# IONIQ6000/av1-go

Hardware: AMD Instinct MI355X
Metric: encoded 4K30 frames/sec (whole node) at fixed QP; PSNR-Y delta vs libaom (higher is better)
Workload: dtype u16

## Files before the change

av1-go_amd/csrc/av1_entropy_kernels.hip:

```cpp
#include <string.h>
#include <vector>
#include "av1_ops_cdfs.hpp"
#include "av1_ops8.hpp"
#include "av1mi_internal.hpp"

namespace av1mi {
using namespace av1ops;

struct Av1EntLaunch {
  FrameView fv;
  int nframes, sbr_n, sbc_n;
  BlockInfo *info;
  op_t *ops; uint32_t ops_cap;
  uint32_t *grouped; uint32_t grouped_cap;
  uint16_t *slot_total, *slot_base;
  uint16_t *rec;
  uint32_t *nops;
  uint8_t *slots; uint32_t slot_cap;
  uint32_t *tile_size;
  uint64_t *tile_off;
  uint32_t *status;
  uint8_t *out; uint64_t out_cap;
  const uint16_t *cdf_image; int cdf_words;
  SlotTable tab;
  const uint16_t *cdf_image32; SlotTable tab32;
  const uint8_t *lr_on_frame;
  int sb_rows32, band, nslots;
};

template <int kKey = -1> __device__ __forceinline__ FrameView frame_view(const Av1EntLaunch &L, int f) {
  FrameView v = L.fv;
  const long nb = (long)v.w8 * v.h8;
  if (kKey < 0 ? v.key != 0 : kKey != 0) { v.y_mode += nb * f; v.uv_mode += nb * f; }
  else { v.mv += nb * 2 * f; v.skip += nb * f; }
  v.lev_y += nb * 64 * f; v.lev_u += nb * 16 * f; v.lev_v += nb * 16 * f;
  v.info = L.info + nb * f;
  if (L.lr_on_frame) for (int p = 0; p < 3; p++) v.lr_on[p] = v.lr_on[p] && L.lr_on_frame[f * 3 + p];
  return v;
}

__global__ __launch_bounds__(256) void k_av1_info(Av1EntLaunch L) {
  const long nb = (long)L.fv.w8 * L.fv.h8, i = (long)blockIdx.x * 256 + threadIdx.x;
  if (i >= nb * L.nframes) return;
  const int f = (int)(i / nb), b = (int)(i - (long)f * nb);
  const FrameView v = frame_view<0>(L, f);
  BlockInfo o = {};
  inter_mode_decision(v, b / v.w8, b % v.w8, &o);
  L.info[nb * f + b] = o;
}

struct TileWave {
  template <class T> using Var = LaneVar<T, 1>;
  template <class F> __device__ __forceinline__ void each(F f) { f((int)threadIdx.x); __syncthreads(); }
  __device__ __forceinline__ int scan(Var<int> &v) {
    const int lane = (int)threadIdx.x, x = v.v[0];
    int inc = x;
#pragma unroll
    for (int d = 1; d < 64; d <<= 1) {
      const int y = __shfl_up(inc, d, 64);
      if (lane >= d) inc += y;
    }
    v.v[0] = inc - x;
    return __shfl(inc, 63, 64);
  }
  __device__ __forceinline__ int first(Var<int> &v) { return __shfl(v.v[0], 0, 64); }
};

__global__ __launch_bounds__(64) __attribute__((amdgpu_waves_per_eu(2, 8))) void k_av1_tokens(Av1EntLaunch L) {
  const int tiles = L.sbr_n * L.sbc_n, t = blockIdx.x, f = t / tiles, tt = t - f * tiles, sbr = tt / L.sbc_n, sbc = tt - sbr * L.sbc_n;
  if (sbr < L.sb_rows32) return;
  const FrameView v = frame_view(L, f);
  __shared__ Tile8Mem S;
  const int below = tiles - L.sb_rows32 * L.sbc_n;
  uint16_t *rec = L.rec + ((size_t)f * below + (tt - (tiles - below))) * kBlocksPerTile * kBlockRecords;
  TileWave w;
  const int n = tok_tile8(w, S, v, sbr, sbc, rec, L.ops + (size_t)t * L.ops_cap, L.ops_cap, L.grouped + (size_t)t * L.grouped_cap,
                          L.slot_total + (size_t)t * S_MAX, L.slot_base + (size_t)t * S_MAX);
  if (threadIdx.x == 0) {
    if (n < 0) atomicOr(L.status, 1u);
    L.nops[t] = n < 0 ? 0u : (uint32_t)n;
  }
}

__global__ __launch_bounds__(64) void k_av1_tokens32(Av1EntLaunch L) {
  __shared__ Tile32Mem S;
  const int tiles = L.sbr_n * L.sbc_n, band = L.sb_rows32 * L.sbc_n, f = blockIdx.x / band, tt = blockIdx.x - f * band, sbr = tt / L.sbc_n, sbc = tt - sbr * L.sbc_n;
  const size_t t = (size_t)f * tiles + tt;
  const FrameView v = frame_view<1>(L, f);
  TileWave w;
  const int n = tok_tile32(w, S, v, sbr, sbc, L.ops + t * L.ops_cap, L.ops_cap, L.grouped + t * L.grouped_cap, L.slot_total + t * S_MAX, L.slot_base + t * S_MAX);
  if (threadIdx.x == 0) {
    if (n < 0) atomicOr(L.status, 1u);
    L.nops[t] = n < 0 ? 0u : (uint32_t)n;
  }
}

__global__ __launch_bounds__(64) void k_av1_chains(Av1EntLaunch L, int ntiles_all, int ngroups) {
  const int xcd = blockIdx.x & 7, j = blockIdx.x >> 3, nslots = L.nslots;
  const int g = (j / nslots) * 8 + xcd, sl = j - (j / nslots) * nslots, lane = threadIdx.x, t = g * 64 + lane;
  if (g >= ngroups) return;
  __shared__ __attribute__((aligned(16))) uint16_t s_big[64 * 16];
  const int n = L.tab.nsym[sl], off = L.tab.off[sl];
  int cnt = 0, base = 0;
  bool mine = t < ntiles_all;
  if (mine && L.band) { const int tiles = L.sbr_n * L.sbc_n, sbr = (t % tiles) / L.sbc_n; mine = (sbr < L.sb_rows32) == (L.band == 1); }
  if (mine) { cnt = L.slot_total[(size_t)t * S_MAX + sl]; base = L.slot_base[(size_t)t * S_MAX + sl]; }
  if (!__any(cnt > 0)) return;
  const size_t tt = t < ntiles_all ? (size_t)t : 0;
  op_t *list = L.ops + tt * L.ops_cap;
  const uint32_t *grouped = L.grouped + tt * L.grouped_cap + base;
  if (n <= 4) {
    const uint32_t *iw = reinterpret_cast<const uint32_t *>(L.cdf_image) + (off >> 1);
    uint64_t cdf = (uint64_t)iw[0] | ((uint64_t)iw[1] << 32);
    const uint4 *g4 = reinterpret_cast<const uint4 *>(grouped);
    const uint4 z = make_uint4(0, 0, 0, 0);
    uint4 c0 = cnt > 0 ? g4[0] : z, c1 = cnt > 4 ? g4[1] : z, c2 = cnt > 8 ? g4[2] : z, c3 = cnt > 12 ? g4[3] : z;
    auto four = [&](const uint4 &v, int e) {
      if (e < cnt) list[v.x >> 4] = small_step(cdf, (int)(v.x & 15), n);
      if (e + 1 < cnt) list[v.y >> 4] = small_step(cdf, (int)(v.y & 15), n);
      if (e + 2 < cnt) list[v.z >> 4] = small_step(cdf, (int)(v.z & 15), n);
      if (e + 3 < cnt) list[v.w >> 4] = small_step(cdf, (int)(v.w & 15), n);
    };
#pragma unroll 1
    for (int e = 0; e < cnt; e += 16) {
      const uint4 *nx = g4 + (e >> 2) + 4;
      const uint4 n0 = e + 16 < cnt ? nx[0] : z, n1 = e + 20 < cnt ? nx[1] : z, n2 = e + 24 < cnt ? nx[2] : z, n3 = e + 28 < cnt ? nx[3] : z;
      four(c0, e); four(c1, e + 4); four(c2, e + 8); four(c3, e + 12);
      c0 = n0; c1 = n1; c2 = n2; c3 = n3;
    }
  } else {
    uint16_t *cdf = s_big + lane * 16;
    {
      const uint4 *iw = reinterpret_cast<const uint4 *>(L.cdf_image + off);
      uint4 *d = reinterpret_cast<uint4 *>(cdf);
      d[0] = iw[0];
      d[1] = n > 8 ? iw[1] : make_uint4(0, 0, 0, 0);
    }
#pragma unroll 1
    for (int e = 0; e < cnt; e++) {
      const uint32_t v = grouped[e];
      const int s = (int)(v & 15);
      list[v >> 4] = s >= kSplitHorz ? split_tuple(cdf, s) : big_step(cdf, s, n);
    }
  }
}

constexpr int kRingOps = 64, kLaneWords = kRingOps * 2 + Coder::kStage + 8;

__global__ __launch_bounds__(64) void k_av1_code(Av1EntLaunch L, int ntiles_all) {
  __shared__ __attribute__((aligned(16))) uint16_t s_lane[64 * kLaneWords];
  const int lane = threadIdx.x, t = blockIdx.x * 64 + lane;
  const bool live = t < ntiles_all;
  uint32_t *ring = reinterpret_cast<uint32_t *>(s_lane + lane * kLaneWords);
  Coder c;
  c.init(L.slots + (size_t)(live ? t : 0) * L.slot_cap, (int)L.slot_cap, s_lane + lane * kLaneWords + kRingOps * 2);
  const int n = live ? (int)L.nops[t] : 0;
  const uint4 *ops4 = reinterpret_cast<const uint4 *>(L.ops + (size_t)(live ? t : 0) * L.ops_cap);
  uint4 r0, r1, r2, r3, r4, r5, r6, r7;
  r0 = r1 = r2 = r3 = r4 = r5 = r6 = r7 = make_uint4(0, 0, 0, 0);
  int w = 0;
  bool pend = false;
  auto request = [&]() {
    const uint4 *p = ops4 + (w >> 2);
    if (w < n) r0 = p[0];
    if (w + 4 < n) r1 = p[1];
    if (w + 8 < n) r2 = p[2];
    if (w + 12 < n) r3 = p[3];
    if (w + 16 < n) r4 = p[4];
    if (w + 20 < n) r5 = p[5];
    if (w + 24 < n) r6 = p[6];
    if (w + 28 < n) r7 = p[7];
    pend = w < n;
  };
  auto take = [&]() {
    uint4 *q = reinterpret_cast<uint4 *>(ring + (w & 32));
    q[0] = r0; q[1] = r1; q[2] = r2; q[3] = r3; q[4] = r4; q[5] = r5; q[6] = r6; q[7] = r7;
    w += 32;
  };
  request();
  if (pend) { take(); request(); }
  int i = 0, lit_left = 0;
  uint32_t op = ring[0], op_next = ring[1], op_next2 = ring[2];
  for (;;) {
    if (!__any(lit_left > 0 || i < n)) break;
    if (__any((pend && w - i < 24) || c.ns >= Coder::kStage - 8)) {
      if (pend && w - i <= 32) { take(); request(); }
      c.spill();
    }
#pragma unroll
    for (int q = 0; q < 8; q++) {
      if (lit_left > 0 || i < n) {
        const uint32_t fetched = ring[(i + 3) & (kRingOps - 1)];
        uint32_t tup = op;
        if (lit_left == 0 && (op >> 31)) lit_left = (int)((op >> 27) & 15);
        if (lit_left > 0) {
          lit_left--;
          tup = (op >> lit_left) & 1 ? (1u << 19) | (256u << 9) : (2u << 19) | (512u << 9) | 256u;
        }
        c.encode_tuple(tup);
        if (lit_left == 0) { i++; op = op_next; op_next = op_next2; op_next2 = fetched; }
      }
    }
  }
  if (!live) return;
  int sz = n ? c.finish() : -1;
  if (sz < 0) { if (n) atomicOr(L.status, 2u); sz = 0; }
  L.tile_size[t] = (uint32_t)sz;
}

__global__ __launch_bounds__(1024) void k_av1_scan(Av1EntLaunch L, int ntiles_all) {
// ... 17 lines not shown
  }
}
__global__ __launch_bounds__(64) void k_av1_gather(Av1EntLaunch L) {
  const int t = blockIdx.x;
  const uint32_t n = L.tile_size[t];
  const uint64_t off = L.tile_off[t];
  if (off + n > L.out_cap) return;
  const uint8_t *src = L.slots + (size_t)t * L.slot_cap;
  uint8_t *dst = L.out + off;
  const uint32_t head = min(n, (uint32_t)((16 - (reinterpret_cast<uintptr_t>(dst) & 15)) & 15)), body = (n - head) >> 4, tail0 = head + (body << 4);
  if (threadIdx.x < head) dst[threadIdx.x] = src[threadIdx.x];
  for (uint32_t i = threadIdx.x; i < body; i += 64) {
    uint4 v;
    __builtin_memcpy(&v, src + head + 16 * i, 16);
    *reinterpret_cast<uint4 *>(dst + head + 16 * i) = v;
  }
  if (tail0 + threadIdx.x < n) dst[tail0 + threadIdx.x] = src[tail0 + threadIdx.x];
}

hipError_t launch_av1_front(av1mi_ctx *ctx, const Av1EntLaunch &L, hipStream_t s) {
  const long nb = (long)L.fv.w8 * L.fv.h8 * L.nframes;
  const int ntiles_all = L.sbr_n * L.sbc_n * L.nframes, ngroups = (ntiles_all + 63) / 64;
  ProfToken t = ctx_prof_begin(ctx, AV1MI_K_ENTROPY_TOKENS, s);
  if (!L.fv.key) hipLaunchKernelGGL(k_av1_info, dim3((unsigned)((nb + 255) / 256)), dim3(256), 0, s, L);
  if (L.sb_rows32 < L.sbr_n) hipLaunchKernelGGL(k_av1_tokens, dim3((unsigned)ntiles_all), dim3(64), 0, s, L);
  if (L.sb_rows32) hipLaunchKernelGGL(k_av1_tokens32, dim3((unsigned)(L.sb_rows32 * L.sbc_n * L.nframes)), dim3(64), 0, s, L);
  ctx_prof_end(ctx, t, s);
  t = ctx_prof_begin(ctx, AV1MI_K_ENTROPY_CHAINS, s);
  Av1EntLaunch C = L;
  C.nslots = L.fv.key ? S_KEY_END : S_INTER_END; C.band = L.sb_rows32 ? 2 : 0;
  if (L.sb_rows32 < L.sbr_n) hipLaunchKernelGGL(k_av1_chains, dim3((unsigned)(((ngroups + 7) / 8) * 8 * C.nslots)), dim3(64), 0, s, C, ntiles_all, ngroups);
  if (L.sb_rows32) {
    C.nslots = K_END; C.band = 1; C.tab = L.tab32; C.cdf_image = L.cdf_image32;
    hipLaunchKernelGGL(k_av1_chains, dim3((unsigned)(((ngroups + 7) / 8) * 8 * C.nslots)), dim3(64), 0, s, C, ntiles_all, ngroups);
  }
  ctx_prof_end(ctx, t, s);
  return hipGetLastError();
}
hipError_t launch_av1_back(av1mi_ctx *ctx, const Av1EntLaunch &L, hipStream_t s) {
  const int ntiles_all = L.sbr_n * L.sbc_n * L.nframes;
  ProfToken t = ctx_prof_begin(ctx, AV1MI_K_ENTROPY, s);
  hipLaunchKernelGGL(k_av1_code, dim3((unsigned)((ntiles_all + 63) / 64)), dim3(64), 0, s, L, ntiles_all);
  ctx_prof_end(ctx, t, s);
  t = ctx_prof_begin(ctx, AV1MI_K_ENTROPY_PACK, s);
  hipLaunchKernelGGL(k_av1_scan, dim3(1), dim3(1024), 0, s, L, ntiles_all);
  hipLaunchKernelGGL(k_av1_gather, dim3((unsigned)ntiles_all), dim3(64), 0, s, L);
  ctx_prof_end(ctx, t, s);
  return hipGetLastError();
}

}

struct av1mi_av1ent_state {
  void *info = nullptr, *ops[2] = { nullptr, nullptr }, *nops[2] = { nullptr, nullptr }, *grouped = nullptr, *slot_tb = nullptr, *rec = nullptr, *slots = nullptr, *tile_off = nullptr, *status = nullptr;
  size_t info_b = 0, ops_b[2] = { 0, 0 }, nops_b[2] = { 0, 0 }, grouped_b = 0, slot_tb_b = 0, rec_b = 0, slots_b = 0, off_b = 0;
  hipEvent_t lists_ready[2] = { nullptr, nullptr }, lists_free[2] = { nullptr, nullptr };
  bool free_recorded[2] = { false, false };
  unsigned long jobs = 0;
  av1mi::Av1EntLaunch pending[2];
  uint64_t *pending_total[2] = { nullptr, nullptr };
  bool pending_valid[2] = { false, false };
  size_t last_tiles = 0;
  uint16_t *d_image[2][4] = {};
  uint16_t *d_image32[4] = {};
  av1ops::SlotTable tab32;
  int image_words[2] = { 0, 0 };
  av1ops::SlotTable tab[2];
};

namespace {
int grow(av1mi_ctx *ctx, void **p, size_t *have, size_t need) {
  if (*have >= need) return AV1MI_OK;
  if (*p) (void)hipFree(*p);
  *p = nullptr; *have = 0;
  if (hipMalloc(p, need) != hipSuccess) return av1mi::ctx_fail(ctx, AV1MI_E_NOMEM, "AV1 entropy scratch: hipMalloc(%zu) failed", need);
  *have = need;
  return AV1MI_OK;
}
}

extern "C" {

uint32_t av1mi_av1_entropy_ops_per_tile(void) { return 32768; }
uint32_t av1mi_av1_entropy_slot_bytes(void) { return 16384; }

}

int av1mi::av1_entropy_front(av1mi_ctx *ctx, const av1mi_av1_entropy_job *j, hipStream_t front, int *ticket) {
  if (!ctx || !ticket) return AV1MI_E_INVAL;
  *ticket = -1;
  if (!j) return av1mi::ctx_fail(ctx, AV1MI_E_INVAL, "null job");
  if (hipSetDevice(av1mi::ctx_device(ctx)) != hipSuccess) return av1mi::ctx_fail(ctx, AV1MI_E_DEVICE, "hipSetDevice failed");
  if (j->width <= 0 || j->height <= 0 || (j->width & 7) || (j->height & 7) || j->width > 4096 || j->height > 4096)
    return av1mi::ctx_fail(ctx, AV1MI_E_INVAL, "frame %dx%d must be a multiple of 8, at most 4096x4096", j->width, j->height);
  if (j->nframes < 0 || j->nframes > 4096 || j->base_q_idx < 1 || j->base_q_idx > 255) return av1mi::ctx_fail(ctx, AV1MI_E_INVAL, "bad nframes / base_q_idx");
  const void *need[] = { j->d_lev_y, j->d_lev_u, j->d_lev_v, j->d_out, j->d_tile_size, j->d_total, j->key ? (const void *)j->d_modes_y : (const void *)j->d_mvs,
                         j->key ? (const void *)j->d_modes_uv : (const void *)j->d_skip };
  for (const void *p : need) if (!p) return av1mi::ctx_fail(ctx, AV1MI_E_INVAL, "null device pointer");
  if (j->nframes == 0) return AV1MI_OK;
  av1mi_av1ent_state *st = av1mi::ctx_av1ent(ctx);
  if (!st) return av1mi::ctx_fail(ctx, AV1MI_E_NOMEM, "AV1 entropy state");
  const int key = j->key ? 1 : 0, qcat = av1ops::q_category(j->base_q_idx);
  if (!st->d_image[key][qcat]) {
    av1ops::SlotTable tab;
    const std::vector<uint16_t> img = av1ops::default_slot_image(key != 0, qcat, &tab);
    st->tab[key] = tab; st->image_words[key] = tab.words;
    if (hipMalloc((void **)&st->d_image[key][qcat], img.size() * 2) != hipSuccess ||
        hipMemcpy(st->d_image[key][qcat], img.data(), img.size() * 2, hipMemcpyHostToDevice) != hipSuccess)
      return av1mi::ctx_fail(ctx, AV1MI_E_DEVICE, "uploading the default CDF image failed");
  }
  if (j->key_rows32 && (!key || (j->key_rows32 & 63) || j->key_rows32 > j->height || (j->width & 31)))
    return av1mi::ctx_fail(ctx, AV1MI_E_INVAL, "key_rows32 %d: whole superblock rows of a key frame whose width is a multiple of 32", j->key_rows32);
  if (j->key_rows32 && !st->d_image32[qcat]) {
    const std::vector<uint16_t> img = av1ops::default_slot_image_k32(qcat, &st->tab32);
    if (hipMalloc((void **)&st->d_image32[qcat], img.size() * 2) != hipSuccess ||
        hipMemcpy(st->d_image32[qcat], img.data(), img.size() * 2, hipMemcpyHostToDevice) != hipSuccess)
      return av1mi::ctx_fail(ctx, AV1MI_E_DEVICE, "uploading the default CDF image failed");
  }
  av1mi::Av1EntLaunch L;
  memset(&L, 0, sizeof(L));
  L.sb_rows32 = j->key_rows32 / 64;
  if (j->key_rows32) { L.tab32 = st->tab32; L.cdf_image32 = st->d_image32[qcat]; }
  L.fv.w8 = j->width / 8; L.fv.h8 = j->height / 8; L.fv.key = key;
  L.fv.y_mode = j->d_modes_y; L.fv.uv_mode = j->d_modes_uv; L.fv.mv = j->d_mvs; L.fv.skip = j->d_skip;
  L.fv.lev_y = j->d_lev_y; L.fv.lev_u = j->d_lev_u; L.fv.lev_v = j->d_lev_v;
  for (int p = 0; p < 3; p++) {
    L.fv.lr_on[p] = j->lr_on[p] != 0;
    const int vh = j->visible_height ? j->visible_height : j->height, vw = j->visible_width ? j->visible_width : j->width;
    const int ph = p ? (vh + 1) / 2 : vh, pw = p ? (vw + 1) / 2 : vw;
    L.fv.lr_rows[p] = (ph + 32) / 64 > 1 ? (ph + 32) / 64 : 1; L.fv.lr_cols[p] = (pw + 32) / 64 > 1 ? (pw + 32) / 64 : 1;
  }
  memcpy(L.fv.lr_unit[0], j->lr_unit_y, 8); memcpy(L.fv.lr_unit[1], j->lr_unit_uv, 8);
  L.nframes = j->nframes; L.sbr_n = (L.fv.h8 + 7) / 8; L.sbc_n = (L.fv.w8 + 7) / 8;
  const size_t nb = (size_t)L.fv.w8 * L.fv.h8 * j->nframes, nt = (size_t)L.sbr_n * L.sbc_n * j->nframes;
  L.ops_cap = av1mi_av1_entropy_ops_per_tile(); L.slot_cap = av1mi_av1_entropy_slot_bytes();
  L.grouped_cap = L.ops_cap + av1ops::kListAlign * av1ops::S_MAX;
  const int par = (int)(st->jobs++ & 1);
  st->last_tiles = nt;
  int rc;
  if ((rc = grow(ctx, &st->info, &st->info_b, nb * sizeof(av1ops::BlockInfo))) ||
      (rc = grow(ctx, &st->ops[par], &st->ops_b[par], nt * L.ops_cap * sizeof(av1ops::op_t))) || (rc = grow(ctx, &st->nops[par], &st->nops_b[par], nt * 4)) ||
      (rc = grow(ctx, &st->grouped, &st->grouped_b, nt * L.grouped_cap * sizeof(uint32_t))) ||
      (rc = grow(ctx, &st->slot_tb, &st->slot_tb_b, nt * av1ops::S_MAX * 4)) ||
      (rc = grow(ctx, &st->rec, &st->rec_b, (size_t)(L.sbr_n - L.sb_rows32) * L.sbc_n * j->nframes * av1ops::kBlocksPerTile * av1ops::kBlockRecords * sizeof(uint16_t))) ||
      (rc = grow(ctx, &st->slots, &st->slots_b, nt * L.slot_cap)) || (rc = grow(ctx, &st->tile_off, &st->off_b, (nt + 1) * 8)))
    return rc;
  L.info = (av1ops::BlockInfo *)st->info; L.ops = (av1ops::op_t *)st->ops[par]; L.nops = (uint32_t *)st->nops[par]; L.grouped = (uint32_t *)st->grouped;
  L.slot_total = (uint16_t *)st->slot_tb; L.slot_base = L.slot_total + nt * av1ops::S_MAX; L.rec = (uint16_t *)st->rec; L.slots = (uint8_t *)st->slots;
  L.tile_off = (uint64_t *)st->tile_off;
  L.tile_size = j->d_tile_size; L.out = j->d_out; L.out_cap = j->out_cap;
  L.status = (uint32_t *)(j->d_total + 1);
  L.cdf_image = st->d_image[key][qcat]; L.cdf_words = st->image_words[key]; L.tab = st->tab[key];
  L.lr_on_frame = j->d_lr_on;
#define E_HIP(call) do { const hipError_t e_ = (call); if (e_ != hipSuccess) return av1mi::ctx_fail(ctx, AV1MI_E_DEVICE, "%s: %s", #call, hipGetErrorString(e_)); } while (0)
  for (hipEvent_t *ev : { &st->lists_ready[par], &st->lists_free[par] }) if (!*ev) E_HIP(hipEventCreateWithFlags(ev, hipEventDisableTiming));
  if (st->free_recorded[par]) E_HIP(hipStreamWaitEvent(front, st->lists_free[par], 0));
  E_HIP(hipMemsetAsync(j->d_total, 0, 16, front));
  E_HIP(av1mi::launch_av1_front(ctx, L, front));
  E_HIP(hipEventRecord(st->lists_ready[par], front));
  st->pending[par] = L; st->pending_total[par] = j->d_total; st->pending_valid[par] = true;
  *ticket = par;
  return AV1MI_OK;
}

int av1mi::av1_entropy_back(av1mi_ctx *ctx, int ticket, hipStream_t back) {
  if (!ctx || ticket < 0 || ticket > 1) return AV1MI_E_INVAL;
  av1mi_av1ent_state *st = av1mi::ctx_av1ent(ctx);
  if (!st || !st->pending_valid[ticket]) return av1mi::ctx_fail(ctx, AV1MI_E_INVAL, "no entropy job pending under this ticket");
  const av1mi::Av1EntLaunch &L = st->pending[ticket];
  const size_t nt = (size_t)L.sbr_n * L.sbc_n * L.nframes;
  E_HIP(hipStreamWaitEvent(back, st->lists_ready[ticket], 0));
  E_HIP(av1mi::launch_av1_back(ctx, L, back));
  E_HIP(hipMemcpyAsync(st->pending_total[ticket], L.tile_off + nt, 8, hipMemcpyDeviceToDevice, back));
  E_HIP(hipEventRecord(st->lists_free[ticket], back)); st->free_recorded[ticket] = true;
  st->pending_valid[ticket] = false;
#undef E_HIP
  return AV1MI_OK;
}

int av1mi::av1_entropy_submit(av1mi_ctx *ctx, const av1mi_av1_entropy_job *j, hipStream_t front, hipStream_t back) {
  int ticket = -1;
  const int rc = av1_entropy_front(ctx, j, front, &ticket);
  if (rc != AV1MI_OK || ticket < 0) return rc;
  return av1_entropy_back(ctx, ticket, back);
}

extern "C" {

int av1mi_av1_entropy_encode_on(av1mi_ctx *ctx, const av1mi_av1_entropy_job *j, void *stream_handle) {
  if (!ctx) return AV1MI_E_INVAL;
  hipStream_t s = stream_handle ? (hipStream_t)stream_handle : av1mi::ctx_stream(ctx);
  return av1mi::av1_entropy_submit(ctx, j, s, s);
}

int av1mi_av1_entropy_encode(av1mi_ctx *ctx, const av1mi_av1_entropy_job *j) { return av1mi_av1_entropy_encode_on(ctx, j, nullptr); }

int av1mi_av1_entropy_last_list_words(av1mi_ctx *ctx, uint64_t *words) {
  if (!ctx || !words) return AV1MI_E_INVAL;
  *words = 0;
  av1mi_av1ent_state *st = av1mi::ctx_av1ent(ctx);
  if (!st || !st->jobs || !st->last_tiles) return AV1MI_OK;
  if (hipSetDevice(av1mi::ctx_device(ctx)) != hipSuccess || hipDeviceSynchronize() != hipSuccess) return av1mi::ctx_fail(ctx, AV1MI_E_DEVICE, "synchronising failed");
  std::vector<uint32_t> n(st->last_tiles);
  if (hipMemcpy(n.data(), st->nops[(st->jobs - 1) & 1], n.size() * 4, hipMemcpyDeviceToHost) != hipSuccess) return av1mi::ctx_fail(ctx, AV1MI_E_DEVICE, "reading the list sizes failed");
  for (uint32_t v : n) *words += v;
  return AV1MI_OK;
}

}

namespace av1mi {
void av1ent_free(av1mi_av1ent_state *st) {
  if (!st) return;
  for (void *p : { st->info, st->ops[0], st->ops[1], st->nops[0], st->nops[1], st->grouped, st->slot_tb, st->rec, st->slots, st->tile_off }) if (p) (void)hipFree(p);
  for (hipEvent_t ev : { st->lists_ready[0], st->lists_ready[1], st->lists_free[0], st->lists_free[1] }) if (ev) (void)hipEventDestroy(ev);
  for (auto &k : st->d_image) for (uint16_t *p : k) if (p) (void)hipFree(p);
  for (uint16_t *p : st->d_image32) if (p) (void)hipFree(p);
  delete st;
}
av1mi_av1ent_state *av1ent_new() { return new (std::nothrow) av1mi_av1ent_state(); }
}
```

av1-go_amd/csrc/av1_ops32.hpp:

```cpp
#pragma once
#include "av1_ops.hpp"

namespace av1ops {

enum SlotK32 : int {
  K_SKIP = 0,
  K_PART32 = 1,
  K_PART64 = 2,
  K_USE_WIENER = 3,
  K_TXB_SKIP_Y = 4,
  K_TXB_SKIP_C = 5,
  K_EOB_Y = 8,
  K_EOB_C = 9,
  K_EOBX_Y = 10,
  K_EOBX_C = 19,
  K_DC_SIGN_Y = 26,
  K_DC_SIGN_C = 29,
  K_BASE_EOB_Y = 32,
  K_BASE_EOB_C = 36,
  K_BASE_Y = 40,
  K_BASE_C = 66,
  K_BR_Y = 92,
  K_BR_C = 113,
  K_KF_Y_MODE = 134,
// ... 210 lines not shown
      uint8_t *col = reinterpret_cast<uint8_t *>(S.round) + lane;
      for (int rs = 0; rs < kRoundSlots; rs++) col[rs * (kRoundStride * 4)] = 0;
      if (lane < nr) {
        CountSink32 k = { col, chroma, 0 };
        R::pass1(k, S, lev, b, p, eob, nr - 1 - lane);
        c = k.n;
      }
    }
    opened[lane] = o; n[lane] = c + o;
  });
  const int words1 = w.scan(n);
  typename W::template Var<RoundCounts> cnt;
  const int nd = (nr + 3) >> 2;
  w.each([&](int lane) {
    if (lane >= kRoundSlots) return;
    RoundCounts &c = cnt[lane];
    AV1_UNROLL
    for (int q = 0; q < kLanes32 / 4; q++) c.w[q] = q < nd ? S.round[lane * kRoundStride + q] : 0u;
  });
  w.each([&](int lane) {
    if (lane >= kRoundSlots) return;
    const RoundCounts &c = cnt[lane];
    const int slot = round_slot_global(lane, chroma);
    uint32_t run = S.run[slot];
    AV1_UNROLL
    for (int q = 0; q < kLanes32 / 4; q++) {
      if (q >= nd) continue;
      const uint32_t u = c.w[q], p0 = run, p1 = p0 + (u & 0xFF), p2 = p1 + ((u >> 8) & 0xFF), p3 = p2 + ((u >> 16) & 0xFF);
      run = p3 + (u >> 24);
      S.round[lane * kRoundStride + 2 * q] = p0 | (p1 << 16); S.round[lane * kRoundStride + 2 * q + 1] = p2 | (p3 << 16);
    }
    S.run[slot] = run;
  });
  w.each([&](int lane) {
    if (lane >= nr) return;
    EmitSink32 k = { reinterpret_cast<u16a *>(S.round) + lane, chroma, words + n[lane] + opened[lane], list, grouped };
    R::pass1(k, S, lev, b, p, eob, nr - 1 - lane);
  });
  words += words1;
  w.each([&](int lane) {
    WordSink32 k = { 0 };
    if (lane < nr) R::pass2(k, S, lev, b, p, eob, lane);
    n[lane] = k.n;
  });
  const int words2 = w.scan(n);
  w.each([&](int lane) {
    if (lane >= nr) return;
    DirectSink32 k = { S.run, words + n[lane], list, grouped };
    R::pass2(k, S, lev, b, p, eob, lane);
  });
  return words + words2;
}

template <class W>
AV1_HD int tok_tile32(W &w, Tile32Mem &S, const FrameView &f, int sbr, int sbc, op_t *list, uint32_t ops_cap, uint32_t *grouped, uint16_t *slot_total,
                      uint16_t *slot_base) {
  typedef typename W::template Var<int> LaneInt;
  const bool half = sbc * 8 + 4 >= f.w8;
  w.each([&](int lane) {
    fill_scan_tables32(&S.scan, lane, kLanes32);
    for (int i = lane; i < kTile32MagBytes / 4; i += kLanes32) reinterpret_cast<u32a *>(S.mag)[i] = 0;
    for (int i = lane; i < K_END; i += kLanes32) S.run[i] = 0;
    if (lane < kBlocks32 * 3) { S.eob[lane] = 0; S.cul[lane] = 0; }
  });
  w.each([&](int lane) {
    AV1_UNROLL
    for (int b = 0; b < kBlocks32; b++) {
      if (half && (b & 1)) continue;
      const long i = block_index32(f, sbr, sbc, b);
      int eob = 0, cul = 0;
      MagMap<32> Y(tile_scratch32(S, b, 0));
      eob = Y.load8(f.lev_y + i * 1024, lane, &cul);
      eob = imax(eob, Y.load8(f.lev_y + i * 1024, lane + kLanes32, &cul));
      if (cul) { AV1_SHARED_MAX(&S.eob[b * 3], eob); AV1_SHARED_ADD(&S.cul[b * 3], cul); }
      const int p = 1 + (lane >> 5);
      MagMap<16> C(tile_scratch32(S, b, p));
      cul = 0;
      eob = C.load8((p == 1 ? f.lev_u : f.lev_v) + i * 256, lane & 31, &cul);
      if (cul) { AV1_SHARED_MAX(&S.eob[b * 3 + p], eob); AV1_SHARED_ADD(&S.cul[b * 3 + p], cul); }
    }
  });
  LaneInt n;
  w.each([&](int lane) {
    TotalSink32 k = { S.run, 0 };
    for (int b = 0; b < kBlocks32; b++) {
      if (half && (b & 1)) continue;
      tok_tb32_total<32>(f, k, S, lane, sbr, sbc, b, 0, half);
      tok_tb32_total<16>(f, k, S, lane, sbr, sbc, b, 1, half);
      tok_tb32_total<16>(f, k, S, lane, sbr, sbc, b, 2, half);
    }
    n[lane] = k.n;
  });
  const int words = w.scan(n);
  enum { kOwn = (K_END + kLanes32 - 1) / kLanes32 };
  w.each([&](int lane) {
    int mine = 0;
    for (int q = 0; q < kOwn; q++) if (lane * kOwn + q < K_END) mine += (int)((S.run[lane * kOwn + q] + kListAlign - 1) & ~(uint32_t)(kListAlign - 1));
    n[lane] = mine;
  });
  const int entries = w.scan(n);
  const bool fits = (uint32_t)words <= ops_cap && entries <= 65535;
  w.each([&](int lane) {
    uint32_t run = (uint32_t)n[lane];
    for (int q = 0; q < kOwn; q++) {
      const int sl = lane * kOwn + q;
      if (sl >= K_END) break;
      const uint32_t tot = S.run[sl];
      slot_total[sl] = (uint16_t)(fits ? tot : 0u); slot_base[sl] = (uint16_t)(fits ? run : 0u);
      S.run[sl] = run;
      run += (tot + kListAlign - 1) & ~(uint32_t)(kListAlign - 1);
    }
    for (int sl = K_END + lane; sl < S_MAX; sl += kLanes32) { slot_total[sl] = 0; slot_base[sl] = 0; }
  });
  if (!fits) return -1;
  int at = 0;
  for (int b = 0; b < kBlocks32; b++) {
    if (half && (b & 1)) continue;
    at = tok_tb32_emit<32>(w, S, f, sbr, sbc, b, 0, half, at, list, grouped);
    at = tok_tb32_emit<16>(w, S, f, sbr, sbc, b, 1, half, at, list, grouped);
    at = tok_tb32_emit<16>(w, S, f, sbr, sbc, b, 2, half, at, list, grouped);
  }
  return at;
}

}
```

av1-go_amd/csrc/av1_ops8.hpp:

```cpp
#pragma once
#include "av1_ops32.hpp"

namespace av1ops {

enum { kLanes8 = kBlocksPerTile, kReplaySlots = (S_MAX + 1) / 2, kOwn8 = (S_MAX + kLanes8 - 1) / kLanes8 };
static_assert(2 * kReplaySlots >= S_MAX && S_MAX <= 256 && kOwn8 * kLanes8 >= S_MAX && 4 * kLanes8 >= S_MAX, "rows are bytes; two passes cover every slot");

struct Tile8Mem {
  union {
    struct { uint8_t cnt[S_MAX * kBlocksPerTile]; alignas(16) uint8_t mag[kBlocksPerTile * kMagBytes]; } p1;
    uint16_t pos[kReplaySlots * kBlocksPerTile];
  };
  uint16_t total[S_MAX], base[S_MAX];
  uint8_t row[(S_MAX + 3) & ~3];
  uint8_t sums[kBlocksPerTile];
  ScanTables scan;
};
struct SlotCounts8 { uint32_t w[kOwn8][kBlocksPerTile / 4]; };

AV1_HD void replay_block8(const uint16_t *rec, int nrec, uint16_t *pos, const uint8_t *row, int blk, int first, op_t *list, uint32_t *grouped, int row_lo,
                          bool literals) {
  int n = first;
  for (int i0 = 0; i0 < nrec; i0 += 8) {
    struct alignas(16) R8 { uint32_t w[4]; } q = *reinterpret_cast<const R8 *>(rec + i0);
    AV1_UNROLL
    for (int j = 0; j < 8; j++, n++) {
      if (i0 + j >= nrec) break;
      const unsigned r = (q.w[j >> 1] >> (16 * (j & 1))) & 0xFFFFu;
      if (r & 0x8000u) { if (literals) list[n] = op_lit((int)((r >> 11) & 15), r & 0x7FFu); }
      else {
        const unsigned rw = (unsigned)row[r >> 4] - (unsigned)row_lo;
        if (rw < (unsigned)kReplaySlots) { uint16_t &p = pos[rw * kBlocksPerTile + blk]; grouped[p] = ((uint32_t)n << 4) | (r & 15u); p++; }
      }
    }
  }
}

template <class W>
AV1_HD int tok_tile8(W &w, Tile8Mem &S, const FrameView &f, int sbr, int sbc, uint16_t *rec, op_t *list, uint32_t ops_cap, uint32_t *grouped,
                     uint16_t *slot_total, uint16_t *slot_base) {
  typedef typename W::template Var<int> LaneInt;
  const int nslots = f.key ? S_KEY_END : S_INTER_END;
  w.each([&](int lane) {
    for (int i = lane; i < S_MAX * kBlocksPerTile / 4; i += kLanes8) reinterpret_cast<u32a *>(S.p1.cnt)[i] = 0;
    if (lane == 0) fill_scan_tables(&S.scan);
    int bx, by;
    demorton8((unsigned)lane, &bx, &by);
    const int r8 = sbr * 8 + by, c8 = sbc * 8 + bx;
    S.sums[by * 8 + bx] = (uint8_t)(r8 < f.h8 && c8 < f.w8 ? block_levels_summary(f, r8 * f.w8 + c8) : 0u);
  });
  LaneInt nrec, first;
  w.each([&](int lane) {
    const TokScratch ts = { S.p1.mag + lane * kMagBytes, &S.scan };
    Sink k = { rec + (size_t)lane * kBlockRecords, S.p1.cnt, lane, 0, 0, false };
    tok_block(f, k, ts, sbr, sbc, lane, S.sums);
    nrec[lane] = k.nrec;
    first[lane] = k.n | (k.overflow ? 1 << 24 : 0);
  });
  const int sum = w.scan(first), words = sum & 0xFFFFFF;
  bool fits = (uint32_t)words <= ops_cap && !(sum >> 24);
  typename W::template Var<SlotCounts8> cnt;
  if (fits) w.each([&](int lane) {
    SlotCounts8 &c = cnt[lane];
    AV1_UNROLL
    for (int q = 0; q < kOwn8; q++) {
      const int sl = lane + kLanes8 * q;
      int tot = 0;
      AV1_UNROLL
      for (int i = 0; i < kBlocksPerTile / 4; i++) {
        const uint32_t u = sl < nslots ? reinterpret_cast<const u32a *>(S.p1.cnt)[sl * (kBlocksPerTile / 4) + i] : 0u;
        c.w[q][i] = u;
#if defined(__HIP_DEVICE_COMPILE__)
        tot = (int)__builtin_amdgcn_sad_u8(u, 0u, (unsigned)tot);
#else
        tot += (int)((u & 0xFF) + ((u >> 8) & 0xFF) + ((u >> 16) & 0xFF) + (u >> 24));
#endif
      }
      if (sl < S_MAX) S.total[sl] = (uint16_t)tot;
    }
  });
  LaneInt ent, used;
  if (fits) w.each([&](int lane) {
    int e = 0, u = 0;
    for (int q = 0; q < 4; q++) {
      const int sl = 4 * lane + q;
      if (sl < nslots) { e += (S.total[sl] + kListAlign - 1) & ~(kListAlign - 1); u += S.total[sl] != 0; }
    }
    ent[lane] = e; used[lane] = u;
  });
  const int entries = fits ? w.scan(ent) : 0, rows = fits ? w.scan(used) : 0;
  fits = fits && entries <= 65535;
  if (!fits) {
    w.each([&](int lane) { for (int sl = lane; sl < S_MAX; sl += kLanes8) slot_total[sl] = 0; });
    return -1;
  }
  w.each([&](int lane) {
    int run = ent[lane], r = used[lane];
    for (int q = 0; q < 4; q++) {
      const int sl = 4 * lane + q;
      if (sl >= nslots) break;
      const int tot = S.total[sl];
      S.base[sl] = (uint16_t)run; S.row[sl] = (uint8_t)r;
      run += (tot + kListAlign - 1) & ~(kListAlign - 1); r += tot != 0;
    }
  });
  const int npass = rows <= kReplaySlots ? 1 : 2;
  for (int pass = 0; pass < npass; pass++) {
    const int row_lo = pass * kReplaySlots;
    w.each([&](int lane) {
      const SlotCounts8 &c = cnt[lane];
      AV1_UNROLL
      for (int q = 0; q < kOwn8; q++) {
        const int sl = lane + kLanes8 * q;
        if (sl >= S_MAX) continue;
        if (pass == 0) { const bool on = sl < nslots; slot_total[sl] = on ? S.total[sl] : (uint16_t)0; slot_base[sl] = on ? S.base[sl] : (uint16_t)0; }
        if (sl >= nslots || !S.total[sl]) continue;
        const unsigned rw = (unsigned)S.row[sl] - (unsigned)row_lo;
        if (rw >= (unsigned)kReplaySlots) continue;
        int run = S.base[sl];
        AV1_UNROLL
        for (int i = 0; i < kBlocksPerTile / 4; i++) {
          const uint32_t u = c.w[q][i];
          const int p0 = run, p1 = p0 + (int)(u & 0xFF), p2 = p1 + (int)((u >> 8) & 0xFF), p3 = p2 + (int)((u >> 16) & 0xFF);
          run = p3 + (int)(u >> 24);
          u32a *d = reinterpret_cast<u32a *>(S.pos + rw * kBlocksPerTile + 4 * i);
          d[0] = (uint32_t)p0 | ((uint32_t)p1 << 16); d[1] = (uint32_t)p2 | ((uint32_t)p3 << 16);
        }
      }
    });
    w.each([&](int lane) {
      replay_block8(rec + (size_t)lane * kBlockRecords, nrec[lane], S.pos, S.row, lane, first[lane] & 0xFFFFFF, list, grouped, row_lo, pass == 0);
    });
  }
  return words;
}

}
```

av1-go_amd/host/av1_opstream.cpp:

```cpp
#include <algorithm>
#include <cstdio>
#include <cstdlib>
#include <cstring>
#include <string>
#include <vector>
#include "../csrc/av1_ops_cdfs.hpp"
#include "../csrc/av1_ops8.hpp"
#include "av1_bitstream.hpp"

namespace av1mi_host {
namespace av1 {

bool opstream_supported(const av1mi_obu_frame &f, std::string *why) {
  auto no = [&](const char *m) { if (why) *why = m; return false; };
  if (f.cdef_bits || f.reduced_tx_set || f.disable_cdf_update) return no("cdef_bits / reduced_tx_set / disable_cdf_update must be 0");
  if (f.tile_cols_log2 >= 0 || f.tile_rows_log2 >= 0) return no("one superblock per tile only");
  if (f.angle_y || f.angle_uv || f.cfl_alpha || f.tx_type || f.is_inter) return no("angle deltas, chroma from luma, transform types and intra blocks in inter frames are host-writer only");
  if (f.frame_type == 0 && f.skip) return no("key frames are coded with skip = 0");
  for (int p = 0; p < 3; p++) if (f.lr_type[p] > 1) return no("Wiener restoration only");
  if (f.lr_unit_shift || f.lr_uv_shift) return no("64x64 restoration units only");
  return true;
}

namespace {
// ... 34 lines not shown
  }
}
bool lr_units_of(const av1mi_obu_frame &f, av1ops::FrameView *v, std::string *err) {
  for (int p = 0; p < 3; p++) {
    if (!v->lr_on[p]) continue;
    const int8_t *u = f.lr_units[p];
    const size_t n = (size_t)v->lr_rows[p] * v->lr_cols[p];
    for (size_t i = 1; i < n; i++) if (memcmp(u, u + i * 8, 8)) { if (err) *err = "restoration units must be uniform per plane"; return false; }
    if (p == 2 && v->lr_on[1] && memcmp(u, f.lr_units[1], 8)) { if (err) *err = "U and V restoration units must be equal"; return false; }
    memcpy(v->lr_unit[p ? 1 : 0], u, 8);
  }
  return true;
}
}

bool opstream_tiles(const av1mi_obu_frame &f, std::vector<std::vector<uint8_t>> *tiles, std::string *err, int key_rows32) {
  using namespace av1ops;
  if (!opstream_supported(f, err)) return false;
  if (key_rows32 && (f.frame_type != 0 || (key_rows32 & 63) || key_rows32 > f.height || (f.width & 31))) { if (err) *err = "bad 32x32 band"; return false; }
  FrameView v;
  frame_view_of(f, &v);
  std::vector<uint8_t> zskip;
  if (!v.key && !v.skip) { zskip.assign((size_t)v.w8 * v.h8, 0); v.skip = zskip.data(); }
  if (!lr_units_of(f, &v, err)) return false;
  const size_t nb = (size_t)v.w8 * v.h8;
  std::vector<BlockInfo> info(nb);
  v.info = info.data();
  for (size_t b = 0; b < nb; b++) memset(&info[b], 0, sizeof(BlockInfo));
  if (!v.key) for (int r = 0; r < v.h8; r++) for (int c = 0; c < v.w8; c++) inter_mode_decision(v, r, c, &info[(size_t)r * v.w8 + c]);
  const int qcat = q_category(f.base_q_idx);
  SlotTable tab;
  const std::vector<uint16_t> image = default_slot_image(v.key != 0, qcat, &tab);
  const int sbr_n = (v.h8 + 7) / 8, sbc_n = (v.w8 + 7) / 8;
  tiles->assign((size_t)sbr_n * sbc_n, {});
  const int nslots = v.key ? S_KEY_END : S_INTER_END;
  std::vector<Tile8Mem> mem8(1);
  std::vector<uint16_t> rec((size_t)kBlocksPerTile * kBlockRecords);
  const uint32_t ops_cap8 = 1u << 20;
  std::vector<op_t> list8(ops_cap8);
  std::vector<uint32_t> grouped8(65536 + kListAlign);
  const bool stats = getenv("AV1MI_TOK_STATS") != nullptr;
  int st_rec = 0, st_cnt = 0, st_ops = 0, st_over = 0; long st_ops_sum = 0;
  SlotTable tab32;
  const std::vector<uint16_t> image32 = key_rows32 ? default_slot_image_k32(qcat, &tab32) : std::vector<uint16_t>();
  std::vector<Tile32Mem> mem32(key_rows32 ? 1 : 0);
  const uint32_t ops_cap32 = 1u << 20;
  std::vector<op_t> list32(key_rows32 ? ops_cap32 : 0);
  std::vector<uint32_t> grouped32(key_rows32 ? 65536 : 0);
  for (int sbr = 0; sbr < sbr_n; sbr++)
    for (int sbc = 0; sbc < sbc_n; sbc++) {
      if (sbr * 64 < key_rows32) {
        WaveLoop wave;
        uint16_t base[S_MAX], total[S_MAX];
        const int words = tok_tile32(wave, mem32[0], v, sbr, sbc, list32.data(), ops_cap32, grouped32.data(), total, base);
        if (words < 0) { if (err) *err = "tile too large for 16-bit entry positions"; return false; }
        std::vector<op_t> list(list32.begin(), list32.begin() + words);
        if (!code_list(list, grouped32, K_END, total, base, tab32, image32.data(), &(*tiles)[(size_t)sbr * sbc_n + sbc], err)) return false;
        continue;
      }
      WaveLoop wave;
      uint16_t base[S_MAX], total[S_MAX];
      const int words = tok_tile8(wave, mem8[0], v, sbr, sbc, rec.data(), list8.data(), ops_cap8, grouped8.data(), total, base);
      if (stats) {
        std::vector<uint8_t> cnt((size_t)S_MAX * kBlocksPerTile, 0);
        const TokScratch ts = { mem8[0].p1.mag, &mem8[0].scan };
        int ops = 0;
        for (int zi = 0; zi < kBlocksPerTile; zi++) {
          Sink k = { rec.data(), cnt.data(), zi, 0, 0, false };
          tok_block(v, k, ts, sbr, sbc, zi, mem8[0].sums);
          st_rec = std::max(st_rec, k.nrec); ops += k.n;
        }
        for (uint8_t c : cnt) st_cnt = std::max(st_cnt, (int)c);
        st_ops = std::max(st_ops, ops); st_ops_sum += ops;
        if (words < 0) { st_over++; continue; }
      }
      if (words < 0) { if (err) *err = "a tile exceeds the tokenizer's capacities (records or symbols of a slot per block, entries per tile)"; return false; }
      std::vector<op_t> list(list8.begin(), list8.begin() + words);
      if (!code_list(list, grouped8, nslots, total, base, tab, image.data(), &(*tiles)[(size_t)sbr * sbc_n + sbc], err)) return false;
    }
  if (stats)
    fprintf(stderr, "[av1mi tok stats] %d tiles: records per block <= %d (capacity %d), symbols of a slot in a block <= %d (255), list words per tile <= %d, mean %.0f; %d tiles over a block capacity\n",
            sbr_n * sbc_n, st_rec, (int)kBlockRecords, st_cnt, st_ops, (double)st_ops_sum / (sbr_n * sbc_n), st_over);
  return true;
}

int opstream_slots() { return av1ops::S_MAX; }

int opstream_tile8(const av1mi_obu_frame &f, int sbr, int sbc, uint32_t ops_cap, uint32_t *list, uint32_t *grouped, uint16_t *slot_total, uint16_t *slot_base,
                   std::string *err) {
  using namespace av1ops;
  if (!opstream_supported(f, err) || sbr < 0 || sbc < 0 || sbr * 64 >= f.height || sbc * 64 >= f.width) return -2;
  FrameView v;
  frame_view_of(f, &v);
  std::vector<uint8_t> zskip;
  if (!v.key && !v.skip) { zskip.assign((size_t)v.w8 * v.h8, 0); v.skip = zskip.data(); }
  if (!lr_units_of(f, &v, err)) return -2;
  std::vector<BlockInfo> info(v.key ? 0 : (size_t)v.w8 * v.h8);
  v.info = info.data();
  if (!v.key) for (int r = 0; r < v.h8; r++) for (int c = 0; c < v.w8; c++) { memset(&info[(size_t)r * v.w8 + c], 0, sizeof(BlockInfo)); inter_mode_decision(v, r, c, &info[(size_t)r * v.w8 + c]); }
  std::vector<Tile8Mem> mem(1);
  std::vector<uint16_t> rec((size_t)kBlocksPerTile * kBlockRecords);
  WaveLoop wave;
  return tok_tile8(wave, mem[0], v, sbr, sbc, rec.data(), list, ops_cap, grouped, slot_total, slot_base);
}

int opstream_tile32(const av1mi_obu_frame &f, int sbr, int sbc, uint32_t ops_cap, uint32_t *list, uint32_t *grouped, uint16_t *slot_total, uint16_t *slot_base,
                    std::string *err) {
  using namespace av1ops;
  if (!opstream_supported(f, err) || f.frame_type != 0 || (f.width & 31) || sbr < 0 || sbc < 0 || (sbr + 1) * 64 > f.height || sbc * 64 >= f.width) return -2;
  FrameView v;
  frame_view_of(f, &v);
  if (!lr_units_of(f, &v, err)) return -2;
  std::vector<Tile32Mem> mem(1);
  WaveLoop wave;
  return tok_tile32(wave, mem[0], v, sbr, sbc, list, ops_cap, grouped, slot_total, slot_base);
}

}
}
```

Measured before the change: 2954.

## Pack per-tile op and grouped lists into a shared pool via atomic cursors

Each tokenizer tile now reserves exactly-sized list and grouped-entry areas from a global pool with atomicAdd on two cursors, rounded to 32-word lines. Tiles no longer start at a fixed ops_cap and grouped_cap stride, so the chains and coder kernels read from offsets stored per tile. The intent is a denser memory footprint and better cache and TLB locality for the later passes, which stream these lists. The cost is atomics, an extra offset indirection, a memset of the cursors per job, and a pool layout that is non-deterministic across runs.

```diff
diff --git a/av1-go_amd/csrc/av1_entropy_kernels.hip b/av1-go_amd/csrc/av1_entropy_kernels.hip
--- a/av1-go_amd/csrc/av1_entropy_kernels.hip
+++ b/av1-go_amd/csrc/av1_entropy_kernels.hip
@@ -13,6 +13,8 @@
   BlockInfo *info;
   op_t *ops; uint32_t ops_cap;
   uint32_t *grouped; uint32_t grouped_cap;
+  uint32_t *list_off, *grouped_off;
+  uint32_t *cursors;
   uint16_t *slot_total, *slot_base;
   uint16_t *rec;
   uint32_t *nops;
@@ -39,6 +41,20 @@
   return v;
 }
 
+constexpr uint32_t kPoolLine = 32;
+struct PoolAreas {
+  const Av1EntLaunch &L; size_t t;
+  __device__ __forceinline__ void reserve(int words, int entries, int *a, int *b) const {
+    const uint32_t la = atomicAdd(L.cursors, ((uint32_t)words + kPoolLine - 1) / kPoolLine), lb = atomicAdd(L.cursors + 1, ((uint32_t)entries + kPoolLine - 1) / kPoolLine);
+    L.list_off[t] = la; L.grouped_off[t] = lb;
+    *a = (int)la; *b = (int)lb;
+  }
+  __device__ __forceinline__ op_t *list(int a) const { return L.ops + (size_t)(uint32_t)a * kPoolLine; }
+  __device__ __forceinline__ uint32_t *grouped(int b) const { return L.grouped + (size_t)(uint32_t)b * kPoolLine; }
+  __device__ __forceinline__ void slot(int sl, uint16_t total, uint16_t base) const { L.slot_total[t * S_MAX + sl] = total; L.slot_base[t * S_MAX + sl] = base; }
+  __device__ __forceinline__ void refuse(int sl) const { L.slot_total[t * S_MAX + sl] = 0; }
+};
+
 __global__ __launch_bounds__(256) void k_av1_info(Av1EntLaunch L) {
   const long nb = (long)L.fv.w8 * L.fv.h8, i = (long)blockIdx.x * 256 + threadIdx.x;
   if (i >= nb * L.nframes) return;
@@ -74,8 +90,8 @@
   const int below = tiles - L.sb_rows32 * L.sbc_n;
   uint16_t *rec = L.rec + ((size_t)f * below + (tt - (tiles - below))) * kBlocksPerTile * kBlockRecords;
   TileWave w;
-  const int n = tok_tile8(w, S, v, sbr, sbc, rec, L.ops + (size_t)t * L.ops_cap, L.ops_cap, L.grouped + (size_t)t * L.grouped_cap,
-                          L.slot_total + (size_t)t * S_MAX, L.slot_base + (size_t)t * S_MAX);
+  PoolAreas out = { L, (size_t)t };
+  const int n = tok_tile8(w, S, v, sbr, sbc, rec, L.ops_cap, out);
   if (threadIdx.x == 0) {
     if (n < 0) atomicOr(L.status, 1u);
     L.nops[t] = n < 0 ? 0u : (uint32_t)n;
@@ -88,7 +104,8 @@
   const size_t t = (size_t)f * tiles + tt;
   const FrameView v = frame_view<1>(L, f);
   TileWave w;
-  const int n = tok_tile32(w, S, v, sbr, sbc, L.ops + t * L.ops_cap, L.ops_cap, L.grouped + t * L.grouped_cap, L.slot_total + t * S_MAX, L.slot_base + t * S_MAX);
+  PoolAreas out = { L, t };
+  const int n = tok_tile32(w, S, v, sbr, sbc, L.ops_cap, out);
   if (threadIdx.x == 0) {
     if (n < 0) atomicOr(L.status, 1u);
     L.nops[t] = n < 0 ? 0u : (uint32_t)n;
@@ -106,9 +123,8 @@
   if (mine && L.band) { const int tiles = L.sbr_n * L.sbc_n, sbr = (t % tiles) / L.sbc_n; mine = (sbr < L.sb_rows32) == (L.band == 1); }
   if (mine) { cnt = L.slot_total[(size_t)t * S_MAX + sl]; base = L.slot_base[(size_t)t * S_MAX + sl]; }
   if (!__any(cnt > 0)) return;
-  const size_t tt = t < ntiles_all ? (size_t)t : 0;
-  op_t *list = L.ops + tt * L.ops_cap;
-  const uint32_t *grouped = L.grouped + tt * L.grouped_cap + base;
+  op_t *list = L.ops + (cnt > 0 ? (size_t)L.list_off[t] * kPoolLine : 0);
+  const uint32_t *grouped = L.grouped + (cnt > 0 ? (size_t)L.grouped_off[t] * kPoolLine : 0) + base;
   if (n <= 4) {
     const uint32_t *iw = reinterpret_cast<const uint32_t *>(L.cdf_image) + (off >> 1);
     uint64_t cdf = (uint64_t)iw[0] | ((uint64_t)iw[1] << 32);
@@ -155,7 +171,7 @@
   Coder c;
   c.init(L.slots + (size_t)(live ? t : 0) * L.slot_cap, (int)L.slot_cap, s_lane + lane * kLaneWords + kRingOps * 2);
   const int n = live ? (int)L.nops[t] : 0;
-  const uint4 *ops4 = reinterpret_cast<const uint4 *>(L.ops + (size_t)(live ? t : 0) * L.ops_cap);
+  const uint4 *ops4 = reinterpret_cast<const uint4 *>(L.ops + (n ? (size_t)L.list_off[t] * kPoolLine : 0));
   uint4 r0, r1, r2, r3, r4, r5, r6, r7;
   r0 = r1 = r2 = r3 = r4 = r5 = r6 = r7 = make_uint4(0, 0, 0, 0);
   int w = 0;
@@ -279,8 +295,8 @@
 }
 
 struct av1mi_av1ent_state {
-  void *info = nullptr, *ops[2] = { nullptr, nullptr }, *nops[2] = { nullptr, nullptr }, *grouped = nullptr, *slot_tb = nullptr, *rec = nullptr, *slots = nullptr, *tile_off = nullptr, *status = nullptr;
-  size_t info_b = 0, ops_b[2] = { 0, 0 }, nops_b[2] = { 0, 0 }, grouped_b = 0, slot_tb_b = 0, rec_b = 0, slots_b = 0, off_b = 0;
+  void *info = nullptr, *ops[2] = { nullptr, nullptr }, *nops[2] = { nullptr, nullptr }, *grouped = nullptr, *grouped_off = nullptr, *slot_tb = nullptr, *rec = nullptr, *slots = nullptr, *tile_off = nullptr, *status = nullptr;
+  size_t info_b = 0, ops_b[2] = { 0, 0 }, nops_b[2] = { 0, 0 }, grouped_b = 0, grouped_off_b = 0, slot_tb_b = 0, rec_b = 0, slots_b = 0, off_b = 0;
   hipEvent_t lists_ready[2] = { nullptr, nullptr }, lists_free[2] = { nullptr, nullptr };
   bool free_recorded[2] = { false, false };
   unsigned long jobs = 0;
@@ -296,6 +312,7 @@
 };
 
 namespace {
+constexpr size_t kCursorBytes = 128;
 int grow(av1mi_ctx *ctx, void **p, size_t *have, size_t need) {
   if (*have >= need) return AV1MI_OK;
   if (*p) (void)hipFree(*p);
@@ -366,14 +383,16 @@
   st->last_tiles = nt;
   int rc;
   if ((rc = grow(ctx, &st->info, &st->info_b, nb * sizeof(av1ops::BlockInfo))) ||
-      (rc = grow(ctx, &st->ops[par], &st->ops_b[par], nt * L.ops_cap * sizeof(av1ops::op_t))) || (rc = grow(ctx, &st->nops[par], &st->nops_b[par], nt * 4)) ||
-      (rc = grow(ctx, &st->grouped, &st->grouped_b, nt * L.grouped_cap * sizeof(uint32_t))) ||
-      (rc = grow(ctx, &st->slot_tb, &st->slot_tb_b, nt * av1ops::S_MAX * 4)) ||
+      (rc = grow(ctx, &st->ops[par], &st->ops_b[par], nt * L.ops_cap * sizeof(av1ops::op_t))) || (rc = grow(ctx, &st->nops[par], &st->nops_b[par], nt * 8)) ||
+      (rc = grow(ctx, &st->grouped, &st->grouped_b, nt * L.grouped_cap * sizeof(uint32_t))) || (rc = grow(ctx, &st->grouped_off, &st->grouped_off_b, nt * 4)) ||
+      (rc = grow(ctx, &st->slot_tb, &st->slot_tb_b, kCursorBytes + nt * av1ops::S_MAX * 4)) ||
       (rc = grow(ctx, &st->rec, &st->rec_b, (size_t)(L.sbr_n - L.sb_rows32) * L.sbc_n * j->nframes * av1ops::kBlocksPerTile * av1ops::kBlockRecords * sizeof(uint16_t))) ||
       (rc = grow(ctx, &st->slots, &st->slots_b, nt * L.slot_cap)) || (rc = grow(ctx, &st->tile_off, &st->off_b, (nt + 1) * 8)))
     return rc;
   L.info = (av1ops::BlockInfo *)st->info; L.ops = (av1ops::op_t *)st->ops[par]; L.nops = (uint32_t *)st->nops[par]; L.grouped = (uint32_t *)st->grouped;
-  L.slot_total = (uint16_t *)st->slot_tb; L.slot_base = L.slot_total + nt * av1ops::S_MAX; L.rec = (uint16_t *)st->rec; L.slots = (uint8_t *)st->slots;
+  L.list_off = L.nops + nt; L.grouped_off = (uint32_t *)st->grouped_off;
+  L.cursors = (uint32_t *)st->slot_tb;
+  L.slot_total = (uint16_t *)((uint8_t *)st->slot_tb + kCursorBytes); L.slot_base = L.slot_total + nt * av1ops::S_MAX; L.rec = (uint16_t *)st->rec; L.slots = (uint8_t *)st->slots;
   L.tile_off = (uint64_t *)st->tile_off;
   L.tile_size = j->d_tile_size; L.out = j->d_out; L.out_cap = j->out_cap;
   L.status = (uint32_t *)(j->d_total + 1);
@@ -383,6 +402,7 @@
   for (hipEvent_t *ev : { &st->lists_ready[par], &st->lists_free[par] }) if (!*ev) E_HIP(hipEventCreateWithFlags(ev, hipEventDisableTiming));
   if (st->free_recorded[par]) E_HIP(hipStreamWaitEvent(front, st->lists_free[par], 0));
   E_HIP(hipMemsetAsync(j->d_total, 0, 16, front));
+  E_HIP(hipMemsetAsync(L.cursors, 0, kCursorBytes, front));
   E_HIP(av1mi::launch_av1_front(ctx, L, front));
   E_HIP(hipEventRecord(st->lists_ready[par], front));
   st->pending[par] = L; st->pending_total[par] = j->d_total; st->pending_valid[par] = true;
@@ -439,7 +459,7 @@
 namespace av1mi {
 void av1ent_free(av1mi_av1ent_state *st) {
   if (!st) return;
-  for (void *p : { st->info, st->ops[0], st->ops[1], st->nops[0], st->nops[1], st->grouped, st->slot_tb, st->rec, st->slots, st->tile_off }) if (p) (void)hipFree(p);
+  for (void *p : { st->info, st->ops[0], st->ops[1], st->nops[0], st->nops[1], st->grouped, st->grouped_off, st->slot_tb, st->rec, st->slots, st->tile_off }) if (p) (void)hipFree(p);
   for (hipEvent_t ev : { st->lists_ready[0], st->lists_ready[1], st->lists_free[0], st->lists_free[1] }) if (ev) (void)hipEventDestroy(ev);
   for (auto &k : st->d_image) for (uint16_t *p : k) if (p) (void)hipFree(p);
   for (uint16_t *p : st->d_image32) if (p) (void)hipFree(p);
diff --git a/av1-go_amd/csrc/av1_ops32.hpp b/av1-go_amd/csrc/av1_ops32.hpp
--- a/av1-go_amd/csrc/av1_ops32.hpp
+++ b/av1-go_amd/csrc/av1_ops32.hpp
@@ -286,9 +286,17 @@
   return words + words2;
 }
 
-template <class W>
-AV1_HD int tok_tile32(W &w, Tile32Mem &S, const FrameView &f, int sbr, int sbc, op_t *list, uint32_t ops_cap, uint32_t *grouped, uint16_t *slot_total,
-                      uint16_t *slot_base) {
+struct CallerAreas {
+  op_t *list_; uint32_t *grouped_; uint16_t *slot_total, *slot_base;
+  AV1_HD void reserve(int, int, int *a, int *b) const { *a = 0; *b = 0; }
+  AV1_HD op_t *list(int) const { return list_; }
+  AV1_HD uint32_t *grouped(int) const { return grouped_; }
+  AV1_HD void slot(int sl, uint16_t total, uint16_t base) const { slot_total[sl] = total; slot_base[sl] = base; }
+  AV1_HD void refuse(int sl) const { slot_total[sl] = 0; }
+};
+
+template <class W, class O>
+AV1_HD int tok_tile32(W &w, Tile32Mem &S, const FrameView &f, int sbr, int sbc, uint32_t ops_cap, O &out) {
   typedef typename W::template Var<int> LaneInt;
   const bool half = sbc * 8 + 4 >= f.w8;
   w.each([&](int lane) {
@@ -340,13 +348,17 @@
       const int sl = lane * kOwn + q;
       if (sl >= K_END) break;
       const uint32_t tot = S.run[sl];
-      slot_total[sl] = (uint16_t)(fits ? tot : 0u); slot_base[sl] = (uint16_t)(fits ? run : 0u);
+      out.slot(sl, (uint16_t)(fits ? tot : 0u), (uint16_t)(fits ? run : 0u));
       S.run[sl] = run;
       run += (tot + kListAlign - 1) & ~(uint32_t)(kListAlign - 1);
     }
-    for (int sl = K_END + lane; sl < S_MAX; sl += kLanes32) { slot_total[sl] = 0; slot_base[sl] = 0; }
+    for (int sl = K_END + lane; sl < S_MAX; sl += kLanes32) out.slot(sl, 0, 0);
   });
   if (!fits) return -1;
+  LaneInt at_list, at_grouped;
+  w.each([&](int lane) { if (lane == 0) out.reserve(words, entries, &at_list[lane], &at_grouped[lane]); });
+  op_t *const list = out.list(w.first(at_list));
+  uint32_t *const grouped = out.grouped(w.first(at_grouped));
   int at = 0;
   for (int b = 0; b < kBlocks32; b++) {
     if (half && (b & 1)) continue;
diff --git a/av1-go_amd/csrc/av1_ops8.hpp b/av1-go_amd/csrc/av1_ops8.hpp
--- a/av1-go_amd/csrc/av1_ops8.hpp
+++ b/av1-go_amd/csrc/av1_ops8.hpp
@@ -36,9 +36,8 @@
   }
 }
 
-template <class W>
-AV1_HD int tok_tile8(W &w, Tile8Mem &S, const FrameView &f, int sbr, int sbc, uint16_t *rec, op_t *list, uint32_t ops_cap, uint32_t *grouped,
-                     uint16_t *slot_total, uint16_t *slot_base) {
+template <class W, class O>
+AV1_HD int tok_tile8(W &w, Tile8Mem &S, const FrameView &f, int sbr, int sbc, uint16_t *rec, uint32_t ops_cap, O &out) {
   typedef typename W::template Var<int> LaneInt;
   const int nslots = f.key ? S_KEY_END : S_INTER_END;
   w.each([&](int lane) {
@@ -91,9 +90,13 @@
   const int entries = fits ? w.scan(ent) : 0, rows = fits ? w.scan(used) : 0;
   fits = fits && entries <= 65535;
   if (!fits) {
-    w.each([&](int lane) { for (int sl = lane; sl < S_MAX; sl += kLanes8) slot_total[sl] = 0; });
+    w.each([&](int lane) { for (int sl = lane; sl < S_MAX; sl += kLanes8) out.refuse(sl); });
     return -1;
   }
+  LaneInt at_list, at_grouped;
+  w.each([&](int lane) { if (lane == 0) out.reserve(words, entries, &at_list[lane], &at_grouped[lane]); });
+  op_t *const list = out.list(w.first(at_list));
+  uint32_t *const grouped = out.grouped(w.first(at_grouped));
   w.each([&](int lane) {
     int run = ent[lane], r = used[lane];
     for (int q = 0; q < 4; q++) {
@@ -113,7 +116,7 @@
       for (int q = 0; q < kOwn8; q++) {
         const int sl = lane + kLanes8 * q;
         if (sl >= S_MAX) continue;
-        if (pass == 0) { const bool on = sl < nslots; slot_total[sl] = on ? S.total[sl] : (uint16_t)0; slot_base[sl] = on ? S.base[sl] : (uint16_t)0; }
+        if (pass == 0) { const bool on = sl < nslots; out.slot(sl, on ? S.total[sl] : (uint16_t)0, on ? S.base[sl] : (uint16_t)0); }
         if (sl >= nslots || !S.total[sl]) continue;
         const unsigned rw = (unsigned)S.row[sl] - (unsigned)row_lo;
         if (rw >= (unsigned)kReplaySlots) continue;
diff --git a/av1-go_amd/host/av1_opstream.cpp b/av1-go_amd/host/av1_opstream.cpp
--- a/av1-go_amd/host/av1_opstream.cpp
+++ b/av1-go_amd/host/av1_opstream.cpp
@@ -110,7 +110,8 @@
       if (sbr * 64 < key_rows32) {
         WaveLoop wave;
         uint16_t base[S_MAX], total[S_MAX];
-        const int words = tok_tile32(wave, mem32[0], v, sbr, sbc, list32.data(), ops_cap32, grouped32.data(), total, base);
+        CallerAreas out = { list32.data(), grouped32.data(), total, base };
+        const int words = tok_tile32(wave, mem32[0], v, sbr, sbc, ops_cap32, out);
         if (words < 0) { if (err) *err = "tile too large for 16-bit entry positions"; return false; }
         std::vector<op_t> list(list32.begin(), list32.begin() + words);
         if (!code_list(list, grouped32, K_END, total, base, tab32, image32.data(), &(*tiles)[(size_t)sbr * sbc_n + sbc], err)) return false;
@@ -118,7 +119,8 @@
       }
       WaveLoop wave;
       uint16_t base[S_MAX], total[S_MAX];
-      const int words = tok_tile8(wave, mem8[0], v, sbr, sbc, rec.data(), list8.data(), ops_cap8, grouped8.data(), total, base);
+      CallerAreas out = { list8.data(), grouped8.data(), total, base };
+      const int words = tok_tile8(wave, mem8[0], v, sbr, sbc, rec.data(), ops_cap8, out);
       if (stats) {
         std::vector<uint8_t> cnt((size_t)S_MAX * kBlocksPerTile, 0);
         const TokScratch ts = { mem8[0].p1.mag, &mem8[0].scan };
@@ -159,7 +161,8 @@
   std::vector<Tile8Mem> mem(1);
   std::vector<uint16_t> rec((size_t)kBlocksPerTile * kBlockRecords);
   WaveLoop wave;
-  return tok_tile8(wave, mem[0], v, sbr, sbc, rec.data(), list, ops_cap, grouped, slot_total, slot_base);
+  CallerAreas out = { list, grouped, slot_total, slot_base };
+  return tok_tile8(wave, mem[0], v, sbr, sbc, rec.data(), ops_cap, out);
 }
 
 int opstream_tile32(const av1mi_obu_frame &f, int sbr, int sbc, uint32_t ops_cap, uint32_t *list, uint32_t *grouped, uint16_t *slot_total, uint16_t *slot_base,
@@ -171,7 +174,8 @@
   if (!lr_units_of(f, &v, err)) return -2;
   std::vector<Tile32Mem> mem(1);
   WaveLoop wave;
-  return tok_tile32(wave, mem[0], v, sbr, sbc, list, ops_cap, grouped, slot_total, slot_base);
+  CallerAreas out = { list, grouped, slot_total, slot_base };
+  return tok_tile32(wave, mem[0], v, sbr, sbc, ops_cap, out);
 }
 
 }
```

Result: faster. 3014, median of 6 (+2.0%).
